# SudhirNikam/cobrix

Measured on AMD Instinct MI355X. Metric: decoded input GB/s + records/s, fixed-len COMP-3 mix, 1-8 MI355X; % HBM peak, higher is better.
Workload: dtype u8; 1 GPU; SYN200: fixed-length 200-byte EBCDIC records, numeric mix (COMP, COMP-3, zoned DISPLAY overpunch, IBM COMP-2, cp037 X(18)) -- BASELINE config C2; records_per_gpu=50000000, input_bytes_per_gpu=10000000000, job_input_bytes=10000000000, output_columns=28, parallelism=dp1, string_layout=Arrow string views (16 B views + long payloads, one pass), occurs_layout=Arrow lists (present elements only), inputs_resident_in_hbm=True

## Files before the change

### cobrix_amd/csrc/cbx_capi.hip

```cpp
#include <hip/hip_runtime.h>

#include <algorithm>
#include <cstdio>
#include <cstring>
#include <functional>
#include <string>
#include <vector>

#include "cbx_kernels.hip"
#include "cbx_select.h"
#include "cbx_text.h"
#include "cbx_hier.h"
#include "cbx_walk.h"
#include "cbx_chain.h"
#include "cbx_filter.h"

using namespace cbx;

static thread_local std::string g_err;

static int fail(int code, const std::string& msg) {
    g_err = msg;
    return code;
}
// ... 58 lines not shown
    std::vector<int32_t> seq_field, seq_slot;
    std::vector<int64_t> seq_tile_cap;
    std::vector<SeqCall> h_seqcall;
    std::vector<int64_t> h_seq_scratch;
    SeqCall* d_seqcall = nullptr;
    uint32_t* d_str_tot = nullptr;  int64_t str_tot_cap = 0;
    int64_t* d_str_excl = nullptr;  int64_t str_excl_cap = 0;
    int64_t* d_block_sums = nullptr; int64_t block_sums_cap = 0;
    uint32_t* d_local = nullptr;    int64_t local_cap = 0;
    uint8_t* d_scratch = nullptr;   int64_t scratch_cap = 0;
    uint64_t* d_stamps = nullptr;
    int64_t jit_min = 262144;
    bool jit_tried[4 * kPre + 5] = {};
    hipFunction_t jit_fn[4 * kPre + 5] = {};
    bool jit_coop[4 * kPre + 5] = {};
    int rec_extent = 0;
    std::string jit_error;
    int last_kind = 0;
    int32_t* d_status = nullptr;
    int num_cus = 256;
    bool walk = false;
    int32_t walk_root = 0, walk_var = 0, walk_n_handlers = 0, walk_depth = 1, walk_max_rec = 0;
    cbx_walk_node* d_wnodes = nullptr;
    std::vector<cbx_walk_node> h_wnodes;
    std::vector<cbx_walk_array> h_warr;
    bool walk_jit_tried = false;
    hipFunction_t walk_jit_fn = nullptr;
    bool chain_jit_tried = false;
    hipFunction_t chain_jit_fn[5] = {};
    bool last_chain_jit = false;
// ... 480 lines not shown
                       (const int64_t*)P->d_block_sums, P->d_str_excl);
    HIP_CHECK(hipGetLastError());
    return CBX_OK;
}

struct CallShape {
    const uint8_t* data; int64_t data_len; const int64_t* rec_off; const int32_t* rec_len;
    int64_t n_rec; int32_t stride; int32_t start_off; int64_t first_record_id;
    const int64_t* rec_id = nullptr;
    const int32_t* rec_seg = nullptr;
    int32_t file_id = -1;
};

static int jit_pro(const cbx_plan* P) { return (P->opts.has_segments ? 1 : 0) | (P->harrays.empty() ? 0 : 2); }

static int launch(cbx_plan* P, const CallShape& c, const cbx_column* columns, int mode, hipStream_t st) {
    const int64_t n_tiles = (c.n_rec + kWave - 1) / kWave;
    KernelArgs a{};
    uintptr_t addr = (uintptr_t)c.data;
    a.base_shift = (int64_t)(addr & 15);
    a.data = (const uint8_t*)(addr & ~(uintptr_t)15);
    a.data_len = c.data_len + a.base_shift;
    a.rec_off = c.rec_off;
    a.rec_len = c.rec_len;
    a.n_rec = c.n_rec;
    a.n_tiles = n_tiles;
    a.pitch = n_tiles * kWave;
    a.stride = c.stride;
    a.start_off = c.start_off;
    a.first_record_id = c.first_record_id;
// ... 201 lines not shown
    hipFunction_t jfn = span_fn;
    int jk = -1;
    if (!span && mode == 0 && P->jit_min >= 0 && c.n_rec >= P->jit_min) {
        const int k = contig ? contig_kp(sdw) : 0;
        if (!P->jit_tried[k]) {
            P->jit_tried[k] = true;
            size_t elems = S.sops.size();
            for (const NumOp& o : S.nops) elems += o.run > 1 ? o.run : 1;
            if (elems > (size_t)kJitMaxOps || S.win.size() > (size_t)kJitMaxWindows)
                P->jit_error = "layout has " + std::to_string(elems) + " elements in " + std::to_string(S.win.size()) +
                               " windows, above the specialised-kernel limits (" + std::to_string(kJitMaxOps) + ", " +
                               std::to_string(kJitMaxWindows) + ")";
            else {
                CoopSplit cs;
                P->jit_coop[k] = jit_coop_of(contig, span, jit_pro(P), str_layout_of(P), S.win, S.nops, S.batches, S.sops, false, &cs);
                P->jit_fn[k] = jit_get(jit_source(contig, k, jit_pro(P), str_layout_of(P), S.win, S.nops, S.batches, S.sops, false), &P->jit_error);
            }
        }
        jfn = P->jit_fn[k];
        jk = k;
    }
    P->last_kind = jfn ? 1 : 0;
    const bool coop = jfn && jk >= 0 && P->jit_coop[jk];
    const size_t lds = coop ? kLutLds + (size_t)a.lds_rows + (size_t)kWavesPerBlock * (a.lds_wave - a.lds_rows) : lds_own;
    if (lds > 160 * 1024) return fail(CBX_E_UNSUPPORTED, "record window does not fit in LDS");
    int blocks_per_cu = (int)std::max<size_t>(1, std::min<size_t>(16, (160 * 1024) / lds));
    int occ = 0;
    const hipError_t oe = jfn ? hipModuleOccupancyMaxActiveBlocksPerMultiprocessor(&occ, jfn, kWave * kWavesPerBlock, lds)
                              : hipOccupancyMaxActiveBlocksPerMultiprocessor(&occ, decode_kernel, kWave * kWavesPerBlock, lds);
    if (oe == hipSuccess && occ > 0) blocks_per_cu = std::min(blocks_per_cu, occ);
    if (!coop && contig && S.sops.size() >= S.nops.size() && S.sops.size() > 0) blocks_per_cu = std::min(blocks_per_cu, 4);
    if (const char* e = getenv("CBX_MAX_BLOCKS_PER_CU")) blocks_per_cu = std::max(1, std::min(blocks_per_cu, atoi(e)));
    const bool piped = P->pipe_peer && mode == 0 && P->packed && P->n_seq > 0;
    if (piped && P->pipe_decode_bpc > 0) blocks_per_cu = std::min(blocks_per_cu, P->pipe_decode_bpc);
    const int64_t blocks_needed = coop ? n_tiles : (n_tiles + kWavesPerBlock - 1) / kWavesPerBlock;
    const int64_t grid = std::min<int64_t>(blocks_needed, (int64_t)P->num_cus * blocks_per_cu);
    const bool prof = P->profiling && mode == 0;
    cbx_plan::CallEvents ce{{nullptr, nullptr, nullptr}};
    if (piped && P->pipe_peer->pipe_done) HIP_CHECK(hipStreamWaitEvent(st, P->pipe_peer->pipe_done, 0));
    if (prof) {
        for (auto& e : ce.e) if (!(e = take_event(P))) return fail(CBX_E_HIP, "hipEventCreate failed");
        HIP_CHECK(hipEventRecord(ce.e[0], st));
    }
    hipFunction_t cfn = nullptr;
    int ck = 0;
    if (mode == 0 && P->packed && P->n_seq > 0 && (contig || span) && P->jit_min >= 0 && c.n_rec >= P->jit_min) {
        const int kp = contig ? contig_kp(sdw) : span_kp;
        const int k = (contig ? 2 : 3) * (kPre + 1) + kp;
        if (!P->jit_tried[k]) {
            P->jit_tried[k] = true;
            std::string err;
            CoopSplit cs;
            P->jit_coop[k] = jit_coop_of(true, span, jit_pro(P), 2, S.win, S.nops, S.batches, S.sops, true, &cs);
            P->jit_fn[k] = jit_get(jit_source(true, kp, jit_pro(P), 2, S.win, S.nops, S.batches, S.sops, span, true),
                                   &err, "cbx_jit_count");
        }
        cfn = P->jit_fn[k];
        ck = k;
    }
    if (mode == 0 && P->packed && P->n_seq > 0 && !cfn && !contig) {
        const int kind = P->last_kind;
        if ((r = launch(P, c, columns, 1, st))) return r;
        P->last_kind = kind;
        if (piped) HIP_CHECK(hipEventRecord(P->pipe_done, st));
    } else if (mode == 0 && P->packed && P->n_seq > 0) {
        KernelArgs ac = a;
        ac.mode = 1;
        size_t clds = lds_own;
        const bool ccoop = cfn && P->jit_coop[ck];
        if (cfn) {
            ac.lds_wave = (a.lds_rows + a.lds_counts + 16 + 15) & ~15;
            clds = 1024 + kLutLds + (ccoop ? (size_t)a.lds_rows + (size_t)kWavesPerBlock * (ac.lds_wave - a.lds_rows)
                                           : (size_t)kWavesPerBlock * ac.lds_wave);
// ... 1868 lines not shown
```

### cobrix_amd/csrc/cbx_decode.h

```cpp
#pragma once
#ifndef __HIPCC_RTC__
#include <hip/hip_runtime.h>
#include <stdint.h>
#endif

#include "cobrix_hip.h"

#define CBX_HD __host__ __device__ __forceinline__
#define CBX_HD_NOINLINE __host__ __device__ __attribute__((noinline))

namespace cbx {

struct U128 {
    uint64_t lo, hi;
};

CBX_HD U128 u128(uint64_t lo, uint64_t hi = 0) { return U128{lo, hi}; }

CBX_HD uint64_t mulhi64(uint64_t a, uint64_t b) {
#if defined(__HIP_DEVICE_COMPILE__)
    return __umul64hi(a, b);
#else
    return (uint64_t)(((unsigned __int128)a * b) >> 64);
#endif
// ... 971 lines not shown
    }
}

constexpr int kStrFastBytes = 32;

CBX_HD void img_bytes32(const uint8_t* img, uint32_t addr, int size, uint32_t w[8]) {
    const uint32_t* p = (const uint32_t*)(img + (addr & ~3u));
    const uint32_t sh = addr & 3u;
    uint32_t r[9];
#pragma unroll
    for (int k = 0; k < 9; k++) r[k] = 4 * k < size + 3 ? p[k] : 0u;
#pragma unroll
    for (int k = 0; k < 8; k++) w[k] = align_bytes(r[k + 1], r[k], sh);
}

CBX_HD uint32_t ctz32(uint32_t x) { return (uint32_t)__builtin_ctz(x); }
CBX_HD uint32_t clz32(uint32_t x) { return (uint32_t)__builtin_clz(x); }
CBX_HD uint32_t popc32(uint32_t x) { return (uint32_t)__builtin_popcount(x); }
CBX_HD uint32_t bits_below(int k) { return k >= 32 ? 0xFFFFFFFFu : ((1u << k) - 1u); }

template <typename LutFn>
CBX_HD void lut_entries32(const uint32_t w[8], int size, LutFn lut, uint32_t ev[kStrFastBytes]) {
#pragma unroll
    for (int j = 0; j < kStrFastBytes; j++) ev[j] = j < size ? lut((w[j >> 2] >> (8 * (j & 3))) & 0xFFu) : 0u;
}

CBX_HD StrSpan string_span32e(int trim, const uint32_t ev[kStrFastBytes], int n, int size) {
    uint32_t keep = 0, m2 = 0, m3 = 0;
#pragma unroll
    for (int j = 0; j < kStrFastBytes; j++) {
// ... 61 lines not shown
```

### cobrix_amd/csrc/cbx_device.h

```cpp
#pragma once
#ifndef __HIPCC_RTC__
#include <hip/hip_runtime.h>
#endif

#include "cbx_internal.h"

#ifndef CBX_DIAG
#define CBX_DIAG 0
#endif

namespace cbx {

__device__ __forceinline__ uint32_t wave_excl_scan32(uint32_t x, int lane, uint32_t& total) {
    uint32_t v = x;
    v += (uint32_t)__builtin_amdgcn_update_dpp(0, (int)v, 0x111, 0xF, 0xF, true);
    v += (uint32_t)__builtin_amdgcn_update_dpp(0, (int)v, 0x112, 0xF, 0xF, true);
    v += (uint32_t)__builtin_amdgcn_update_dpp(0, (int)v, 0x114, 0xF, 0xF, true);
    v += (uint32_t)__builtin_amdgcn_update_dpp(0, (int)v, 0x118, 0xF, 0xF, true);
    const uint32_t r0 = (uint32_t)__builtin_amdgcn_readlane((int)v, 15);
    const uint32_t r1 = (uint32_t)__builtin_amdgcn_readlane((int)v, 31);
    const uint32_t r2 = (uint32_t)__builtin_amdgcn_readlane((int)v, 47);
    const uint32_t r3 = (uint32_t)__builtin_amdgcn_readlane((int)v, 63);
    const int row = lane >> 4;
    v += (row >= 1 ? r0 : 0u) + (row >= 2 ? r1 : 0u) + (row >= 3 ? r2 : 0u);
    total = r0 + r1 + r2 + r3;
    return v - x;
// ... 120 lines not shown
    int avail;
    int seg;
};

template <typename OP>
__device__ __forceinline__ bool odo_present(const CBX_CONST OP* opp, int n_odo, const int32_t* s_cnt, int lane) {
    bool el = true;
    for (int j = 0; j < n_odo; j++) el &= opp->odo_idx[j] < s_cnt[opp->odo_arr[j] * kWave + lane];
    return el;
}

__device__ __forceinline__ uint32_t str_lut(int kind, const uint32_t* s_lut, uint32_t b) {
    return kind == CBX_K_STRING_ASCII ? ascii_lut(b) : s_lut[b];
}

__device__ __forceinline__ StrSpan sop_span(const KernelArgs& a, const StrOp& op, const CBX_CONST StrOp* opp,
                                            const TileCtx& t, const int32_t* s_cnt, int lane, const uint8_t* src,
                                            uint32_t rec_addr, const uint32_t* s_lut, bool& ok, bool fast,
                                            uint32_t ev[kStrFastBytes]) {
    bool el = t.active && (op.segment < 0 || op.segment == t.seg);
    if (op.n_odo) el &= odo_present(opp, op.n_odo, s_cnt, lane);
    const int o = a.start_off + op.eo;
    ok = el && o <= t.avail;
    const int n = ok ? (op.size < t.avail - o ? op.size : t.avail - o) : 0;
    auto lutf = [&](uint32_t b) { return str_lut(op.kind, s_lut, b); };
    if (fast) {
        uint32_t w[8];
        img_bytes32(src, rec_addr + (ok ? (uint32_t)op.eo : 0u), op.size, w);
        lut_entries32(w, op.size, lutf, ev);
        return string_span32e(op.trim, ev, n, op.size);
    }
    StrSpan sp{0, 0, 0};
    if (ok) sp = string_span(op.kind, op.trim, src + rec_addr + (uint32_t)op.eo, n, lutf);
    return sp;
}

__device__ __forceinline__ bool sop_fast(const StrOp& op, bool global) {
    return !global && op.size <= kStrFastBytes && (op.kind == CBX_K_STRING || op.kind == CBX_K_STRING_ASCII);
}

template <int W>
__device__ __forceinline__ void store_w(void* values, int64_t tile, int lane, const Val& x, int out_type) {
    const int w = W ? W : (out_type == CBX_O_I32 || out_type == CBX_O_F32 ? 4 : out_type == CBX_O_DEC128 ? 16 : 8);
// ... 177 lines not shown
                    if (kWide) q0[u] = img_le64_ending(src, end - 8);
                }
            }
#pragma unroll
            for (int u = 0; u < kRunU; u++)
                if (r0 + u < run) run_elem<V, W, kOdo>(a, op, a.nops + i, c, r0 + u, t, ok[u], q1[u], q0[u], s_cnt, lane);
        }
    }
}

template <int V, int W, bool kOdo, int N, typename Sink>
__device__ __forceinline__ void num_group(const KernelArgs& a, const NumOp (&op)[N], int i0, const TileCtx& t,
                                          const uint8_t* src, uint32_t rec_addr, const int32_t* s_cnt, int lane, Sink& sk) {
    constexpr bool kWide = V == V_BCD16 || V == V_ZONED16;
    constexpr bool kRead = V != V_GENERIC;
    const int lim = t.active ? t.avail - a.start_off : -1;
    bool ok[N];
    uint64_t r1[N], r0[N];
#pragma unroll
    for (int u = 0; u < N; u++) {
        ok[u] = op[u].eo + op[u].size <= lim;
        r1[u] = r0[u] = 0;
        if (kRead) {
            const uint32_t end = rec_addr + (ok[u] ? (uint32_t)op[u].eo : 0u) + op[u].size;
            r1[u] = img_le64_ending(src, end);
            if (kWide) r0[u] = img_le64_ending(src, end - 8);
        }
    }
#pragma unroll
    for (int u = 0; u < N; u++) num_one<V, W, kOdo, false>(a, op[u], i0 + u, t, ok[u], r1[u], r0[u], s_cnt, lane, sk);
}

__device__ __forceinline__ uint32_t view_buf(int64_t tile, const StrCall& c) {
// ... 225 lines not shown
        const uint32_t so = __builtin_amdgcn_udot4(lb & 0x02020202u, 0x20100804u, 0u, false);
        nb[g] = __builtin_amdgcn_udot4(lb & 0x03030303u, 0x01010101u, 0u, false);
        wide |= g == 0 ? so >> 3 : so << (4 * g - 3);
        sel[g] = group2_sel(so);
    }
    const int len = (e - b) + (int)popc32(wide & bits_below(e) & ~bits_below(b));
    group2_place(smax, u01, u23, nb, sel, b, len, slot, q, zero_tail);
    return len;
}


__device__ __forceinline__ int str_lane_compose(int kind, int trim, int width, int smax, int eo, int n, bool ok,
                                                const uint8_t* src, uint32_t rec_addr, const uint32_t* s_lut,
                                                uint8_t* s_str, int lane, u32x4 (&q)[kStrNC], bool zero_tail) {
    uint32_t w[8], ev[kStrFastBytes];
    img_bytes32(src, rec_addr + (ok ? (uint32_t)eo : 0u), smax, w);
    const uint32_t lut_a = 0;
    (void)s_lut;
#ifndef CBX_STR_NO_SDWA
    if (kind == CBX_K_STRING) {
#pragma unroll
        for (int j = 0; j < kStrFastBytes; j++)
            ev[j] = j < smax ? lds_ld<uint32_t>(lut_a + ((CBX_DIAG & 32) ? diag_bank(byte_x4(w[j >> 2], j & 3)) : byte_x4(w[j >> 2], j & 3))) : 0u;
    } else {
        lut_entries32(w, smax, [&](uint32_t b) { return ascii_lut(b); }, ev);
    }
#else
    lut_entries32(w, smax, [&](uint32_t b) { return str_lut(kind, s_lut, b); }, ev);
#endif
    uint32_t tr = 0;
#pragma unroll
// ... 58 lines not shown
        }
    }
}

__device__ __forceinline__ u32x4 str_short_view(int len, const u32x4 (&q)[kStrNC]) {
    return u32x4{(uint32_t)len, len > 0 ? q[0].x : 0u, len > 4 ? q[0].y : 0u, len > 8 ? q[0].z : 0u};
}

template <typename Sink>
__device__ __forceinline__ void str_view_fast(const KernelArgs& a, const StrOp& op, const CBX_CONST StrOp* opp, int i,
                                              const StrCall& c, const TileCtx& t, const int32_t* s_cnt,
                                              const uint8_t* src, uint32_t rec_addr, const uint32_t* s_lut,
                                              uint8_t* s_str, int lane, Sink& sk) {
    bool el = t.active && (op.segment < 0 || op.segment == t.seg);
    if (op.n_odo) el &= odo_present(opp, op.n_odo, s_cnt, lane);
    const int o = a.start_off + op.eo;
    const bool ok = el && o <= t.avail;
    const int n = ok ? (op.size < t.avail - o ? op.size : t.avail - o) : 0;
    u32x4 q[kStrNC];
    const int len = str_lane_compose(op.kind, op.trim, op.pad, op.size, op.eo, n, ok, src, rec_addr, s_lut, s_str, lane, q);
    sk.svalid(c, i, t.tile, __ballot(ok));
    const bool lng = len > 12;
    uint32_t tot;
    const uint32_t ex = wave_excl_scan32(lng ? (uint32_t)(len + 3) & ~3u : 0u, lane, tot);
    u32x4 v;
    if (!lng) {
        v = str_short_view(len, q);
    } else {
        str_store_long(gp(c.scratch + t.tile * c.tile_cap + ex), len, op.size * op.pad, q);
        v = u32x4{(uint32_t)len, q[0].x, view_buf(t.tile, c), view_pos(t.tile, c, ex)};
    }
    st_out(gp((u32x4*)c.views) + t.tile * kWave + lane, v);
}

template <typename Sink>
__device__ __forceinline__ void str_view_pair(const KernelArgs& a, const StrOp& A, int ia, const StrCall& ca,
                                              const StrOp& B, int ib, const StrCall& cb, const TileCtx& t,
                                              const uint8_t* src, uint32_t rec_addr, const uint32_t* s_lut,
                                              uint8_t* s_str, int lane, Sink& sk) {
    const bool sa = t.seg == A.segment;
    const int eo = sa ? A.eo : B.eo, size = sa ? A.size : B.size;
    const int smax = A.size > B.size ? A.size : B.size;
    const int o = a.start_off + eo;
    const bool ok = t.active && (sa || t.seg == B.segment) && o <= t.avail;
    const int n = ok ? (size < t.avail - o ? size : t.avail - o) : 0;
    u32x4 q[kStrNC];
    const int len = str_lane_compose(A.kind, A.trim, A.pad, smax, eo, n, ok, src, rec_addr, s_lut, s_str, lane, q);
    sk.svalid(ca, ia, t.tile, __ballot(ok && sa));
    sk.svalid(cb, ib, t.tile, __ballot(ok && !sa));
    const bool lng = len > 12;
    uint32_t tot;
    const uint32_t r4 = lng ? (uint32_t)(len + 3) & ~3u : 0u;
    const uint32_t exb = wave_excl_scan32(sa ? r4 : r4 << 16, lane, tot);
    const uint32_t ex = sa ? exb & 0xFFFFu : exb >> 16;
    u32x4 v;
    if (!lng) {
        v = str_short_view(len, q);
    } else {
// ... 62 lines not shown
    case 3: __builtin_amdgcn_s_waitcnt(0x0F73); break;
    case 4: __builtin_amdgcn_s_waitcnt(0x0F74); break;
    case 5: __builtin_amdgcn_s_waitcnt(0x0F75); break;
    case 6: __builtin_amdgcn_s_waitcnt(0x0F76); break;
    default: __builtin_amdgcn_s_waitcnt(0x0F77); break;
    }
    asm volatile("" ::: "memory");
}


__device__ __forceinline__ int utf8_compose(const KernelArgs& a, const StrOp& op, const CBX_CONST StrOp* opp, const TileCtx& t,
                                            const int32_t* s_cnt, const uint8_t* src, uint32_t rec_addr,
                                            const uint32_t* s_lut, uint8_t* s_str, int lane, bool& ok, u32x4 (&q)[kStrNC]) {
    bool el = t.active && (op.segment < 0 || op.segment == t.seg);
    if (op.n_odo) el &= odo_present(opp, op.n_odo, s_cnt, lane);
    const int o = a.start_off + op.eo;
    ok = el && o <= t.avail;
    const int n = ok ? (op.size < t.avail - o ? op.size : t.avail - o) : 0;
    const int len = str_lane_compose(op.kind, op.trim, op.pad, op.size, op.eo, n, ok, src, rec_addr, s_lut, s_str, lane, q, false);
    return ok ? len : 0;
}

__device__ __forceinline__ int64_t utf8_tile_base(const StrCall& c, const TileCtx& t) {
    const CBX_CONST int64_t* x = (const CBX_CONST int64_t*)c.excl;
    return x[t.tile] - x[0];
}

__device__ __forceinline__ CBX_GLOBAL uint8_t* utf8_offsets(const KernelArgs& a, const StrCall& c, const TileCtx& t, int64_t base,
                                                            uint32_t ex, int len, uint32_t tot, int lane) {
    CBX_GLOBAL int32_t* offs = gp((int32_t*)c.local);
    st_out(offs + t.tile * kWave + lane, (int32_t)(base + ex));
// ... 99 lines not shown
        const uint32_t td = sd[k1];
        CBX_GLOBAL uint8_t* tp = A + 4 * k1;
        if (tb >= 2) st_pay((CBX_GLOBAL uint16_t*)(tp), (uint16_t)td);
        if (tb & 1) tp[tb & 2] = (uint8_t)(td >> (8 * (tb & 2)));
    }
}

struct G2 {
    uint32_t u01[kStrNG], u23[kStrNG], nb[kStrNG];
    uint2 sel[kStrNG];
    int b, e, len;
};

__device__ __forceinline__ void g2_prep(int trim, int smax, int eo, int n, bool ok, const uint8_t* src, uint32_t rec_addr, G2& g) {
    uint32_t w[8], ev[kStrFastBytes];
    img_bytes32(src, rec_addr + (ok ? (uint32_t)eo : 0u), smax, w);
#pragma unroll
    for (int j = 0; j < kStrFastBytes; j++)
        ev[j] = j < smax ? lds_ld<uint32_t>(byte_x4(w[j >> 2], j & 3)) : 0u;
    uint32_t tr = 0;
#pragma unroll
    for (int j = 0; j < kStrFastBytes; j++)
        if (j < smax) tr = __builtin_amdgcn_alignbit(tr, ev[j], 31);
    const uint32_t keep = ~(__builtin_bitreverse32(tr) >> (32 - smax)) & bits_below(n);
    int b = 0, e = n;
    if (trim == CBX_TRIM_LEFT || trim == CBX_TRIM_BOTH) b = keep ? (int)ctz32(keep) : n;
    if (trim == CBX_TRIM_RIGHT || trim == CBX_TRIM_BOTH) e = keep ? 32 - (int)clz32(keep) : b;
    uint32_t wide = 0;
#pragma unroll
    for (int q = 0; q < kStrNG; q++) {
        if (4 * q >= smax) break;
// ... 65 lines not shown
    __builtin_amdgcn_s_waitcnt(0xC07F);
    const uint32_t q_lo = ph ? 1u : 0u, q_hi = end >> 4;
    for (uint32_t q = q_lo + (uint32_t)lane; q < q_hi; q += kWave)
        st_pay((CBX_GLOBAL u32x4*)(A + 16u * q), lds_ld<u32x4>(sb + 16u * q));
    const uint32_t he = end < 16u ? end : 16u;
    if (ph && (uint32_t)lane >= ph && (uint32_t)lane < he) A[lane] = lds_ld<uint8_t>(sb + (uint32_t)lane);
    const uint32_t t0 = 16u * q_hi;
    if (t0 >= 16u * q_lo && t0 + (uint32_t)lane < end && (t0 > 0 || !ph)) A[t0 + lane] = lds_ld<uint8_t>(sb + t0 + (uint32_t)lane);
}

__device__ __forceinline__ void str_utf8_fast2(const KernelArgs& a, const StrOp& op, const CBX_CONST StrOp* opp,
                                               const StrCall& c, const TileCtx& t, const int32_t* s_cnt,
                                               const uint8_t* src, uint32_t rec_addr, uint8_t* s_str, int lane) {
    bool el = t.active && (op.segment < 0 || op.segment == t.seg);
    if (op.n_odo) el &= odo_present(opp, op.n_odo, s_cnt, lane);
    const int o = a.start_off + op.eo;
    const bool ok = el && o <= t.avail;
    const int n = ok ? (op.size < t.avail - o ? op.size : t.avail - o) : 0;
    G2 g;
    g2_prep(op.trim, op.size, op.eo, n, ok, src, rec_addr, g);
    gp(c.validity)[t.tile] = __ballot(ok);
    uint32_t tot;
    const uint32_t ex = wave_excl_scan32((uint32_t)g.len, lane, tot);
    CBX_GLOBAL uint8_t* dst = utf8_offsets(a, c, t, utf8_tile_base(c, t), ex, g.len, tot, lane);
    if (!dst || (CBX_DIAG & 16)) return;
#ifndef CBX_U8_DIRECT
    g2_stage_store(dst, ex, tot, op.size, g, true, s_str, lane);
#else
    g2_store(dst + ex, op.size, g, s_str, lane);
#endif
}
// ... 44 lines not shown

__device__ __forceinline__ void str_utf8_two(const KernelArgs& a, const StrOp& A, const CBX_CONST StrOp* oppA, const StrCall& ca,
                                             const StrOp& B, const CBX_CONST StrOp* oppB, const StrCall& cb,
                                             const TileCtx& t, const int32_t* s_cnt, const uint8_t* src, uint32_t rec_addr,
                                             const uint32_t* s_lut, uint8_t* s_str, int lane) {
    str_utf8_two(a, A, oppA, ca, B, oppB, cb, t, s_cnt, src, rec_addr, s_lut, s_str, lane, utf8_tile_base(ca, t),
                 utf8_tile_base(cb, t));
}

__device__ __forceinline__ void str_utf8_pair(const KernelArgs& a, const StrOp& A, const StrCall& ca, const StrOp& B,
                                              const StrCall& cb, const TileCtx& t, const uint8_t* src, uint32_t rec_addr,
                                              const uint32_t* s_lut, uint8_t* s_str, int lane) {
    const bool sa = t.seg == A.segment;
    const int eo = sa ? A.eo : B.eo, size = sa ? A.size : B.size;
    const int smax = A.size > B.size ? A.size : B.size;
    const int o = a.start_off + eo;
    const bool ok = t.active && (sa || t.seg == B.segment) && o <= t.avail;
    const int n = ok ? (size < t.avail - o ? size : t.avail - o) : 0;
    const bool g2 = A.kind == CBX_K_STRING && A.pad == 2;
    G2 g;
    u32x4 q[kStrNC];
    int len;
    if (g2) {
        g2_prep(A.trim, smax, eo, n, ok, src, rec_addr, g);
        len = g.len;
    } else {
        const int l0 = str_lane_compose(A.kind, A.trim, A.pad, smax, eo, n, ok, src, rec_addr, s_lut, s_str, lane, q, false);
        len = ok ? l0 : 0;
    }
    gp(ca.validity)[t.tile] = __ballot(ok && sa);
    gp(cb.validity)[t.tile] = __ballot(ok && !sa);
// ... 12 lines not shown
        return;
    }
#endif
    if (!d) return;
    if (g2) g2_store(d, smax, g, s_str, lane);
    else utf8_store_direct(d, len, smax * A.pad, q);
}

__device__ __forceinline__ uint8_t count_lut_byte(uint32_t e) {
    return (uint8_t)(((e >> 31) << 7) | ((e >> 24) & 3u));
}

__device__ __forceinline__ int str_count_lane(int trim, int smax, int size, int eo, const uint8_t* src, uint32_t rec_addr, bool ok,
                                              const uint32_t* s_lut) {
    uint32_t w[8];
    img_bytes32(src, rec_addr + (ok ? (uint32_t)eo : 0u), smax, w);
    uint32_t acc = 0, tm = 0;
    const uint32_t lut8 = lds_addr(s_lut);
#pragma unroll
    for (int j = 0; j < kStrFastBytes; j++) {
        if (j < smax) {
            const uint32_t idx = (w[j >> 2] >> (8 * (j & 3))) & 0xFFu;
            const uint32_t e = (uint32_t)(int32_t)lds_ld<int8_t>(lut8 + idx);
            tm = __builtin_amdgcn_alignbit(tm, e, 31);
            acc += j < size ? (e & 0xFFu) : 0u;
        }
    }
    const uint32_t keep = ~__builtin_bitreverse32(tm << (32 - smax)) & bits_below(size);
    const int total = (int)(acc & 127u);
    const bool tl = trim == CBX_TRIM_LEFT || trim == CBX_TRIM_BOTH;
    const bool tr = trim == CBX_TRIM_RIGHT || trim == CBX_TRIM_BOTH;
    if (!ok) return 0;
    if (!keep) return (tl || tr) ? 0 : total;
    const int lead = (int)ctz32(keep), trail = size - (32 - (int)clz32(keep));
    return total - (tl ? lead : 0) - (tr ? trail : 0);
}

__device__ __forceinline__ int str_count_fast(const StrOp& op, const uint8_t* src, uint32_t rec_addr, bool ok,
                                              const uint32_t* s_lut) {
    uint32_t w[8];
    img_bytes32(src, rec_addr + (ok ? (uint32_t)op.eo : 0u), op.size, w);
    uint32_t acc = 0;
    const uint32_t lut8 = lds_addr(s_lut);
    const int size = op.size;
#ifndef CBX_COUNT_B64
    uint32_t tm = 0;
#pragma unroll
    for (int j = 0; j < kStrFastBytes; j++) {
        if (j < size) {
            const uint32_t idx = (w[j >> 2] >> (8 * (j & 3))) & 0xFFu;
            const uint32_t e = (uint32_t)(int32_t)lds_ld<int8_t>(lut8 + ((CBX_DIAG & 32) ? diag_bank(idx) : idx));
            tm = __builtin_amdgcn_alignbit(tm, e, 31);
            acc += e & 0xFFu;
        }
    }
    const uint32_t keep = ~__builtin_bitreverse32(tm << (32 - size)) & bits_below(size);
// ... 22 lines not shown
#endif
    const int total = (int)(acc & 127u);
    const bool tl = op.trim == CBX_TRIM_LEFT || op.trim == CBX_TRIM_BOTH;
    const bool tr = op.trim == CBX_TRIM_RIGHT || op.trim == CBX_TRIM_BOTH;
    if (!ok) return 0;
    if (!keep) return (tl || tr) ? 0 : total;
    const int lead = (int)ctz32(keep), trail = size - (32 - (int)clz32(keep));
    return total - (tl ? lead : 0) - (tr ? trail : 0);
}

__device__ __forceinline__ bool str_count_pair(const KernelArgs& a, const StrOp& A, const StrOp& B, const TileCtx& t,
                                               const uint8_t* src, uint32_t rec_addr, const uint32_t* s_lut, int lane) {
    const bool sa = t.seg == A.segment;
    const int eo = sa ? A.eo : B.eo, size = sa ? A.size : B.size;
    const int smax = A.size > B.size ? A.size : B.size;
    const int o = a.start_off + eo;
    const bool el = t.active && (sa || t.seg == B.segment);
    const bool ok = el && o + size <= t.avail;
    const bool part = el && o <= t.avail && !ok;
    if (A.kind != CBX_K_STRING || __ballot(part)) return false;
    const int len = str_count_lane(A.trim, smax, size, eo, src, rec_addr, ok, s_lut + 256);
    const uint32_t la = sa ? (uint32_t)len : 0u, lb = sa ? 0u : (uint32_t)len;
    uint32_t tot2;
    wave_excl_scan32(la | (lb << 16), lane, tot2);
    if (lane == 0) {
        gp(a.str_tot)[(int64_t)A.seq * a.n_tiles + t.tile] = tot2 & 0xFFFFu;
        gp(a.str_tot)[(int64_t)B.seq * a.n_tiles + t.tile] = tot2 >> 16;
    }
    return true;
}

// ... 6 lines not shown
    const bool fast = sop_fast(op, global);
    if (kView && fast) {
        DirectSink ds;
        if (sk) str_view_fast(a, op, opp, i, c, t, s_cnt, src, rec_addr, s_lut, s_str, lane, *sk);
        else str_view_fast(a, op, opp, i, c, t, s_cnt, src, rec_addr, s_lut, s_str, lane, ds);
        return;
    }
    if (!kView && fast && str_layout(a) == 2 && kmode(a) == 0) {
        str_utf8_fast(a, op, opp, c, t, s_cnt, src, rec_addr, s_lut, s_str, lane);
        return;
    }
#ifdef CBX_COUNT_LUT
    if (!kView && fast && op.kind == CBX_K_STRING) {
        bool el = t.active && (op.segment < 0 || op.segment == t.seg);
        if (op.n_odo) el &= odo_present(opp, op.n_odo, s_cnt, lane);
        const int o = a.start_off + op.eo;
        const bool ok = el && o + op.size <= t.avail;
        const bool part = el && o <= t.avail && !ok;
        if (!__ballot(part)) {
            uint32_t tot;
            wave_excl_scan32((uint32_t)str_count_fast(op, src, rec_addr, ok, s_lut + 256), lane, tot);
            if (lane == 0) gp(a.str_tot)[(int64_t)op.seq * a.n_tiles + t.tile] = tot;
            return;
        }
    }
#endif
    bool ok;
    uint32_t ev[kStrFastBytes];
    const StrSpan sp = sop_span(a, op, opp, t, s_cnt, lane, src, rec_addr, s_lut, ok, fast, ev);
    if (kView) {
        DirectSink ds;
// ... 258 lines not shown
}

template <bool kFramed = true>
__device__ __forceinline__ TileCtx tile_ctx(const KernelArgs& a, int64_t tile, int lane) {
    TileCtx t;
    t.tile = tile;
    t.rec = tile * kWave + lane;
    t.active = t.rec < a.n_rec;
    t.base = a.base_shift;
    t.avail = 0;
    t.seg = -1;
    if (kFramed && a.rec_off) {
        if (t.active) { t.base += a.rec_off[t.rec]; t.avail = a.rec_len[t.rec]; }
    } else if (t.active) {
        t.base += t.rec * (int64_t)a.stride;
        t.avail = a.stride;
    }
    return t;
}

template <bool kSel = true, bool kSeg = true, bool kArr = true>
__device__ __forceinline__ void tile_prologue(const KernelArgs& a, TileCtx& t, const uint8_t* rp, int lane,
                                              const uint32_t* s_lut, int32_t* s_cnt) {
    if (kSel && a.rec_seg) t.seg = t.active ? a.rec_seg[t.rec] : -1;
    else if (kSeg && a.segmap && t.active) t.seg = segment_of(a, s_lut, rp, t.avail);
    if (kSeg && kmode(a) == 0 && a.seg_col >= 0) {
        const DevColumn c = ldc(a.cols + a.seg_col);
        if (t.active) gp((int32_t*)c.values)[t.rec] = t.seg;
        const uint64_t m = __ballot(t.active);
        if (lane == 0) gp(c.validity)[t.tile] = m;
    }
// ... 123 lines not shown
    uint4 buf[KP];
    tile = first_tile<Body>(tile);
    if (tile < a.n_tiles) contig_issue<KP>(a, contig_span(a, tile), lane, buf);
    Stamps st;
    st.init();
    while (tile < a.n_tiles) {
        const ContigSpan sp = contig_span(a, tile);
        contig_store<KP>(a, sp, lane, buf, l.img);
        wave_sync_lds();
        st.mark(0);
        const int64_t next = next_tile<Body>(tile, tstep);
        body.begin(tile);
        if (!kLate) contig_issue<KP>(a, contig_span(a, next), lane, buf);
        st.mark(1);
        TileCtx t = tile_ctx<false>(a, tile, lane);
        const uint32_t rec0 = (uint32_t)(lane * a.cpitch + 4 * sp.mis_dw);
        tile_prologue<false, (kPro & 1) != 0, (kPro & 2) != 0>(a, t, l.img + rec0, lane, l.lut, l.cnt);
        st.mark(2);
        body.pre(a, t, (const uint8_t*)l.img, rec0 + (uint32_t)a.start_off, l, lane, st);
        if (kLate) contig_issue<KP>(a, contig_span(a, next), lane, buf);
        body.post(a, t, (const uint8_t*)l.img, rec0 + (uint32_t)a.start_off, l, lane, st);
        run_end(a, body, tile, lane);
        wave_sync_lds();
        st.mark(5);
        tile = next;
    }
    st.flush(a, lane);
}

template <int KP>
__device__ __forceinline__ void coop_issue(const KernelArgs& a, const ContigSpan& sp, int wid, int lane,
                                           uint4 (&buf)[(KP + kWavesPerBlock - 1) / kWavesPerBlock]) {
    constexpr int KH = (KP + kWavesPerBlock - 1) / kWavesPerBlock;
    int64_t left = a.data_len - sp.a0;
    left = left < 0 ? 0 : (left > (1 << 20) ? (1 << 20) : left);
    const uint64_t base = (uint64_t)(a.data + sp.a0);
// ... 38 lines not shown
    tile = first_tile<Body>(tile);
    if (tile >= a.n_tiles) return;
    coop_issue<KP>(a, contig_span(a, tile), wid, lane, buf);
    coop_put<KP>(a, contig_span(a, tile), wid, lane, buf, l.img);
    Stamps st;
    st.init();
    while (true) {
        __syncthreads();
        st.mark(0);
        const ContigSpan sp = contig_span(a, tile);
        const int64_t next = next_tile<Body>(tile, tstep);
        body.begin(tile);
        coop_issue<KP>(a, contig_span(a, next), wid, lane, buf);
        st.mark(1);
        TileCtx t = tile_ctx<false>(a, tile, lane);
        const uint32_t rec0 = (uint32_t)(lane * a.cpitch + 4 * sp.mis_dw);
        st.mark(2);
        body.template part<kW>(a, t, (const uint8_t*)l.img, rec0 + (uint32_t)a.start_off, l, lane, st);
        run_end(a, body, tile, lane);
        __syncthreads();
        st.mark(5);
        tile = next;
        if (tile >= a.n_tiles) break;
        coop_put<KP>(a, contig_span(a, tile), wid, lane, buf, l.img);
    }
    st.flush(a, lane);
}

__device__ __forceinline__ void span_recs(const KernelArgs& a, int64_t tile, int lane, int64_t& off, int32_t& len) {
    const int64_t r = tile * kWave + lane;
    const int64_t rc = r < a.n_rec ? r : a.n_rec - 1;
    const int64_t o = a.rec_off[rc];
    const int32_t l = a.rec_len[rc];
// ... 105 lines not shown
```

### cobrix_amd/csrc/cbx_internal.h

```cpp
#pragma once
#ifndef __HIPCC_RTC__
#include <hip/hip_runtime.h>
#include <stdint.h>
#endif

#include "cbx_decode.h"
#include "cobrix_hip.h"

#define CBX_CONST __attribute__((address_space(4)))

namespace cbx {

constexpr int kWave = 64;
constexpr int kWavesPerBlock = 2;
constexpr int kGuard = 16;
constexpr int kLutLds = 1024 + 128;
constexpr int kMaxWindowBytes = 1024;
constexpr int kStrStageBytes = 4096;
constexpr int kMaxStrItems = 256;

struct StrOp {
    int32_t eo;
    int32_t size;
    uint8_t kind, trim, n_odo, pad;
// ... 105 lines not shown
    const CBX_CONST DevColumn* cols;
    int32_t n_seq;
    uint32_t* str_tot;
    int32_t* status;
    int32_t* list_len;
    int32_t* list_flag;
    uint64_t* defer_bits;
    int32_t lds_rows;
    int32_t lds_counts;
    int32_t str_stage;
    int32_t lds_wave;
    int32_t dump_stride;
    uint64_t* stamps;
};

}
```

### cobrix_amd/csrc/cbx_jit.h

```cpp
#pragma once
#include <hip/hiprtc.h>

#include <algorithm>
#include <cstdlib>
#include <map>
#include <mutex>
#include <sstream>
#include <string>
#include <utility>
#include <vector>

#include "cbx_jit_src.inc"

namespace cbx {

constexpr int kJitMaxStrUnroll = 16;

static std::string jit_u64(uint64_t v) {
    std::ostringstream o;
    o << "0x" << std::hex << v << "ull";
    return o.str();
}

static void jit_numop(std::ostringstream& o, const NumOp& n) {
// ... 197 lines not shown
    bool runs = false;
    for (const NumOp& op : nops) n_defer = std::max(n_defer, op.defer + 1);
    for (const Batch& b : batches) runs |= b.runs != 0;
    *n_str_words = layout == 1 && getenv("CBX_STR_VWORDS") ? (int)sops.size() : 0;
    return (count || runs || span || getenv("CBX_NO_VWORDS")) ? 0 : (int)nops.size() + n_defer + *n_str_words;
}

static bool jit_coop_of(bool contig, bool span, int pro, int layout, const std::vector<Window>& win, const std::vector<NumOp>& nops,
                        const std::vector<Batch>& batches, const std::vector<StrOp>& sops, bool count, CoopSplit* out) {
    int nsw = 0;
    const int nw = contig ? jit_words(layout, nops, batches, sops, span, count, &nsw) : 0;
    return jit_coop(contig, span, pro, win, nops, batches, sops, count, nw, nsw, out);
}

static std::string jit_source(bool contig, int kp, int pro, int layout, const std::vector<Window>& win, const std::vector<NumOp>& nops,
                              const std::vector<Batch>& batches, const std::vector<StrOp>& sops, bool span, bool count = false) {
    std::ostringstream o;
    const bool view = layout == 1;
    if (const char* d = getenv("CBX_JIT_DEFINES")) {
        std::string s(d);
        for (size_t b = 0; b < s.size();) {
            size_t e = s.find(',', b);
            if (e == std::string::npos) e = s.size();
            std::string m = s.substr(b, e - b);
            const size_t q = m.find('=');
            if (!m.empty()) o << "#define " << (q == std::string::npos ? m : m.substr(0, q) + " " + m.substr(q + 1)) << "\n";
            b = e + 1;
        }
    }
    if (getenv("CBX_STR_NO_SHIFT")) o << "#define CBX_STR_NO_SHIFT 1\n";
    o << "#define CBX_STR_LAYOUT " << layout << "\n";
    o << "#define CBX_MODE " << (count ? 1 : 0) << "\n";
// ... 273 lines not shown
```

Before: 2719 GB/s.

## Specialise JIT decode and count kernels on static record geometry

Adds a small per-plan cache of JIT kernels compiled with record stride, LDS pitch and start offset baked in as compile-time constants. String byte gathers can then use constant-offset loads, and the address arithmetic folds away. The decode kernel is specialised only for string-only layouts, while the count kernel is specialised whenever the batch is contiguous. The cost is extra runtime compilations, up to four per kernel kind, when geometry varies.

```diff
diff --git a/cobrix_amd/csrc/cbx_capi.hip b/cobrix_amd/csrc/cbx_capi.hip
--- a/cobrix_amd/csrc/cbx_capi.hip
+++ b/cobrix_amd/csrc/cbx_capi.hip
@@ -96,6 +96,10 @@
     bool jit_tried[4 * kPre + 5] = {};
     hipFunction_t jit_fn[4 * kPre + 5] = {};
     bool jit_coop[4 * kPre + 5] = {};
+    struct JitStatic { JitGeo geo; hipFunction_t fn = nullptr; };
+    std::vector<JitStatic> jit_geo[4 * kPre + 5];
+    bool jit_spec[4 * kPre + 5] = {};
+    bool jit_gen_tried[4 * kPre + 5] = {};
     int rec_extent = 0;
     std::string jit_error;
     int last_kind = 0;
@@ -606,6 +610,18 @@
 
 static int jit_pro(const cbx_plan* P) { return (P->opts.has_segments ? 1 : 0) | (P->harrays.empty() ? 0 : 2); }
 
+template <typename Src>
+static hipFunction_t jit_static(cbx_plan* P, int k, const JitGeo& geo, const char* name, std::string* err, Src src) {
+    for (const cbx_plan::JitStatic& e : P->jit_geo[k])
+        if (e.geo == geo) return e.fn;
+    if ((int)P->jit_geo[k].size() >= kJitMaxGeo) return nullptr;
+    cbx_plan::JitStatic e;
+    e.geo = geo;
+    e.fn = jit_get(src(&e.geo), err, name);
+    P->jit_geo[k].push_back(e);
+    return e.fn;
+}
+
 static int launch(cbx_plan* P, const CallShape& c, const cbx_column* columns, int mode, hipStream_t st) {
     const int64_t n_tiles = (c.n_rec + kWave - 1) / kWave;
     KernelArgs a{};
@@ -837,11 +853,21 @@
             else {
                 CoopSplit cs;
                 P->jit_coop[k] = jit_coop_of(contig, span, jit_pro(P), str_layout_of(P), S.win, S.nops, S.batches, S.sops, false, &cs);
+                P->jit_spec[k] = true;
+            }
+        }
+        jk = k;
+        if (P->jit_spec[k] && contig && S.nops.empty())
+            jfn = jit_static(P, k, JitGeo{a.stride, a.cpitch, a.start_off}, "cbx_jit_decode", &P->jit_error, [&](const JitGeo* g) {
+                return jit_source(true, k, jit_pro(P), str_layout_of(P), S.win, S.nops, S.batches, S.sops, false, false, g);
+            });
+        if (P->jit_spec[k] && !jfn) {
+            if (!P->jit_gen_tried[k]) {
+                P->jit_gen_tried[k] = true;
                 P->jit_fn[k] = jit_get(jit_source(contig, k, jit_pro(P), str_layout_of(P), S.win, S.nops, S.batches, S.sops, false), &P->jit_error);
             }
-        }
-        jfn = P->jit_fn[k];
-        jk = k;
+            jfn = P->jit_fn[k];
+        }
     }
     P->last_kind = jfn ? 1 : 0;
     const bool coop = jfn && jk >= 0 && P->jit_coop[jk];
@@ -872,14 +898,24 @@
         const int k = (contig ? 2 : 3) * (kPre + 1) + kp;
         if (!P->jit_tried[k]) {
             P->jit_tried[k] = true;
-            std::string err;
             CoopSplit cs;
             P->jit_coop[k] = jit_coop_of(true, span, jit_pro(P), 2, S.win, S.nops, S.batches, S.sops, true, &cs);
-            P->jit_fn[k] = jit_get(jit_source(true, kp, jit_pro(P), 2, S.win, S.nops, S.batches, S.sops, span, true),
-                                   &err, "cbx_jit_count");
-        }
-        cfn = P->jit_fn[k];
+        }
         ck = k;
+        std::string cerr;
+        if (contig)
+            cfn = jit_static(P, k, JitGeo{a.stride, a.cpitch, a.start_off}, "cbx_jit_count", &cerr, [&](const JitGeo* g) {
+                return jit_source(true, kp, jit_pro(P), 2, S.win, S.nops, S.batches, S.sops, false, true, g);
+            });
+        if (!cfn) {
+            if (!P->jit_gen_tried[k]) {
+                P->jit_gen_tried[k] = true;
+                std::string err;
+                P->jit_fn[k] = jit_get(jit_source(true, kp, jit_pro(P), 2, S.win, S.nops, S.batches, S.sops, span, true),
+                                       &err, "cbx_jit_count");
+            }
+            cfn = P->jit_fn[k];
+        }
     }
     if (mode == 0 && P->packed && P->n_seq > 0 && !cfn && !contig) {
         const int kind = P->last_kind;
diff --git a/cobrix_amd/csrc/cbx_decode.h b/cobrix_amd/csrc/cbx_decode.h
--- a/cobrix_amd/csrc/cbx_decode.h
+++ b/cobrix_amd/csrc/cbx_decode.h
@@ -1009,6 +1009,21 @@
     for (int k = 0; k < 8; k++) w[k] = align_bytes(r[k + 1], r[k], sh);
 }
 
+CBX_HD void img_bytes32_at(const uint8_t* rec, int off, int size, uint32_t w[8]) {
+    const uint32_t* p = (const uint32_t*)rec + (off >> 2);
+    const uint32_t sh = (uint32_t)off & 3u;
+    uint32_t r[9];
+#pragma unroll
+    for (int k = 0; k < 9; k++) r[k] = 4 * k < size + 3 ? p[k] : 0u;
+#pragma unroll
+    for (int k = 0; k < 8; k++) w[k] = sh == 0 ? r[k] : align_bytes(r[k + 1], r[k], sh);
+}
+template <int OFF, int SIZE>
+CBX_HD void img_bytes32_c(const uint8_t* rec, uint32_t w[8]) {
+    static_assert(OFF >= 0 && SIZE >= 0 && SIZE <= kStrFastBytes, "a register-path string element");
+    img_bytes32_at(rec, OFF, SIZE, w);
+}
+
 CBX_HD uint32_t ctz32(uint32_t x) { return (uint32_t)__builtin_ctz(x); }
 CBX_HD uint32_t clz32(uint32_t x) { return (uint32_t)__builtin_clz(x); }
 CBX_HD uint32_t popc32(uint32_t x) { return (uint32_t)__builtin_popcount(x); }
diff --git a/cobrix_amd/csrc/cbx_device.h b/cobrix_amd/csrc/cbx_device.h
--- a/cobrix_amd/csrc/cbx_device.h
+++ b/cobrix_amd/csrc/cbx_device.h
@@ -10,6 +10,21 @@
 #endif
 
 namespace cbx {
+
+#if defined(CBX_GEO_STRIDE)
+constexpr bool kGeoStatic = true;
+constexpr int kGeoStride = CBX_GEO_STRIDE, kGeoCpitch = CBX_GEO_CPITCH, kGeoStart = CBX_GEO_START, kGeoLim = CBX_GEO_LIM;
+static_assert(kGeoStride > 0 && kGeoStride % 4 == 0 && kGeoCpitch % 4 == 0 && kGeoCpitch >= kGeoStride &&
+              kGeoLim == kGeoStride - kGeoStart, "static geometry of a contiguous fixed-length batch");
+#else
+constexpr bool kGeoStatic = false;
+constexpr int kGeoStride = 0, kGeoCpitch = 0, kGeoStart = 0, kGeoLim = 0;
+#endif
+__device__ __forceinline__ int geo_stride(const KernelArgs& a) { return kGeoStatic ? kGeoStride : a.stride; }
+__device__ __forceinline__ int geo_cpitch(const KernelArgs& a) { return kGeoStatic ? kGeoCpitch : a.cpitch; }
+__device__ __forceinline__ int geo_start(const KernelArgs& a) { return kGeoStatic ? kGeoStart : a.start_off; }
+__device__ __forceinline__ constexpr bool geo_fits(int eo, int size) { return kGeoStatic && eo >= 0 && eo + size <= kGeoLim; }
+__device__ __forceinline__ const uint8_t* geo_rec(const uint8_t* src, uint32_t rec_addr) { return src + (rec_addr - (uint32_t)kGeoStart); }
 
 __device__ __forceinline__ uint32_t wave_excl_scan32(uint32_t x, int lane, uint32_t& total) {
     uint32_t v = x;
@@ -160,19 +175,24 @@
     return kind == CBX_K_STRING_ASCII ? ascii_lut(b) : s_lut[b];
 }
 
+__device__ __forceinline__ void str_bytes32(const uint8_t* src, uint32_t rec_addr, bool ok, int eo, int size, uint32_t w[8]) {
+    if (geo_fits(eo, size)) img_bytes32_at(geo_rec(src, rec_addr), kGeoStart + eo, size, w);
+    else img_bytes32(src, rec_addr + (ok ? (uint32_t)eo : 0u), size, w);
+}
+
 __device__ __forceinline__ StrSpan sop_span(const KernelArgs& a, const StrOp& op, const CBX_CONST StrOp* opp,
                                             const TileCtx& t, const int32_t* s_cnt, int lane, const uint8_t* src,
                                             uint32_t rec_addr, const uint32_t* s_lut, bool& ok, bool fast,
                                             uint32_t ev[kStrFastBytes]) {
     bool el = t.active && (op.segment < 0 || op.segment == t.seg);
     if (op.n_odo) el &= odo_present(opp, op.n_odo, s_cnt, lane);
-    const int o = a.start_off + op.eo;
+    const int o = geo_start(a) + op.eo;
     ok = el && o <= t.avail;
     const int n = ok ? (op.size < t.avail - o ? op.size : t.avail - o) : 0;
     auto lutf = [&](uint32_t b) { return str_lut(op.kind, s_lut, b); };
     if (fast) {
         uint32_t w[8];
-        img_bytes32(src, rec_addr + (ok ? (uint32_t)op.eo : 0u), op.size, w);
+        str_bytes32(src, rec_addr, ok, op.eo, op.size, w);
         lut_entries32(w, op.size, lutf, ev);
         return string_span32e(op.trim, ev, n, op.size);
     }
@@ -380,9 +400,9 @@
                                           const uint8_t* src, uint32_t rec_addr, const int32_t* s_cnt, int lane, Sink& sk) {
     constexpr bool kWide = V == V_BCD16 || V == V_ZONED16;
     constexpr bool kRead = V != V_GENERIC;
-    const int lim = t.active ? t.avail - a.start_off : -1;
     bool ok[N];
     uint64_t r1[N], r0[N];
+    const int lim = t.active ? t.avail - a.start_off : -1;
 #pragma unroll
     for (int u = 0; u < N; u++) {
         ok[u] = op[u].eo + op[u].size <= lim;
@@ -638,7 +658,7 @@
                                                 const uint8_t* src, uint32_t rec_addr, const uint32_t* s_lut,
                                                 uint8_t* s_str, int lane, u32x4 (&q)[kStrNC], bool zero_tail) {
     uint32_t w[8], ev[kStrFastBytes];
-    img_bytes32(src, rec_addr + (ok ? (uint32_t)eo : 0u), smax, w);
+    str_bytes32(src, rec_addr, ok, eo, smax, w);
     const uint32_t lut_a = 0;
     (void)s_lut;
 #ifndef CBX_STR_NO_SDWA
@@ -727,7 +747,7 @@
                                               uint8_t* s_str, int lane, Sink& sk) {
     bool el = t.active && (op.segment < 0 || op.segment == t.seg);
     if (op.n_odo) el &= odo_present(opp, op.n_odo, s_cnt, lane);
-    const int o = a.start_off + op.eo;
+    const int o = geo_start(a) + op.eo;
     const bool ok = el && o <= t.avail;
     const int n = ok ? (op.size < t.avail - o ? op.size : t.avail - o) : 0;
     u32x4 q[kStrNC];
@@ -754,7 +774,7 @@
     const bool sa = t.seg == A.segment;
     const int eo = sa ? A.eo : B.eo, size = sa ? A.size : B.size;
     const int smax = A.size > B.size ? A.size : B.size;
-    const int o = a.start_off + eo;
+    const int o = geo_start(a) + eo;
     const bool ok = t.active && (sa || t.seg == B.segment) && o <= t.avail;
     const int n = ok ? (size < t.avail - o ? size : t.avail - o) : 0;
     u32x4 q[kStrNC];
@@ -847,7 +867,7 @@
                                             const uint32_t* s_lut, uint8_t* s_str, int lane, bool& ok, u32x4 (&q)[kStrNC]) {
     bool el = t.active && (op.segment < 0 || op.segment == t.seg);
     if (op.n_odo) el &= odo_present(opp, op.n_odo, s_cnt, lane);
-    const int o = a.start_off + op.eo;
+    const int o = geo_start(a) + op.eo;
     ok = el && o <= t.avail;
     const int n = ok ? (op.size < t.avail - o ? op.size : t.avail - o) : 0;
     const int len = str_lane_compose(op.kind, op.trim, op.pad, op.size, op.eo, n, ok, src, rec_addr, s_lut, s_str, lane, q, false);
@@ -977,7 +997,7 @@
 
 __device__ __forceinline__ void g2_prep(int trim, int smax, int eo, int n, bool ok, const uint8_t* src, uint32_t rec_addr, G2& g) {
     uint32_t w[8], ev[kStrFastBytes];
-    img_bytes32(src, rec_addr + (ok ? (uint32_t)eo : 0u), smax, w);
+    str_bytes32(src, rec_addr, ok, eo, smax, w);
 #pragma unroll
     for (int j = 0; j < kStrFastBytes; j++)
         ev[j] = j < smax ? lds_ld<uint32_t>(byte_x4(w[j >> 2], j & 3)) : 0u;
@@ -1073,7 +1093,7 @@
                                                const uint8_t* src, uint32_t rec_addr, uint8_t* s_str, int lane) {
     bool el = t.active && (op.segment < 0 || op.segment == t.seg);
     if (op.n_odo) el &= odo_present(opp, op.n_odo, s_cnt, lane);
-    const int o = a.start_off + op.eo;
+    const int o = geo_start(a) + op.eo;
     const bool ok = el && o <= t.avail;
     const int n = ok ? (op.size < t.avail - o ? op.size : t.avail - o) : 0;
     G2 g;
@@ -1148,7 +1168,7 @@
     const bool sa = t.seg == A.segment;
     const int eo = sa ? A.eo : B.eo, size = sa ? A.size : B.size;
     const int smax = A.size > B.size ? A.size : B.size;
-    const int o = a.start_off + eo;
+    const int o = geo_start(a) + eo;
     const bool ok = t.active && (sa || t.seg == B.segment) && o <= t.avail;
     const int n = ok ? (size < t.avail - o ? size : t.avail - o) : 0;
     const bool g2 = A.kind == CBX_K_STRING && A.pad == 2;
@@ -1191,7 +1211,7 @@
 __device__ __forceinline__ int str_count_lane(int trim, int smax, int size, int eo, const uint8_t* src, uint32_t rec_addr, bool ok,
                                               const uint32_t* s_lut) {
     uint32_t w[8];
-    img_bytes32(src, rec_addr + (ok ? (uint32_t)eo : 0u), smax, w);
+    str_bytes32(src, rec_addr, ok, eo, smax, w);
     uint32_t acc = 0, tm = 0;
     const uint32_t lut8 = lds_addr(s_lut);
 #pragma unroll
@@ -1216,7 +1236,7 @@
 __device__ __forceinline__ int str_count_fast(const StrOp& op, const uint8_t* src, uint32_t rec_addr, bool ok,
                                               const uint32_t* s_lut) {
     uint32_t w[8];
-    img_bytes32(src, rec_addr + (ok ? (uint32_t)op.eo : 0u), op.size, w);
+    str_bytes32(src, rec_addr, ok, op.eo, op.size, w);
     uint32_t acc = 0;
     const uint32_t lut8 = lds_addr(s_lut);
     const int size = op.size;
@@ -1269,7 +1289,7 @@
     const bool sa = t.seg == A.segment;
     const int eo = sa ? A.eo : B.eo, size = sa ? A.size : B.size;
     const int smax = A.size > B.size ? A.size : B.size;
-    const int o = a.start_off + eo;
+    const int o = geo_start(a) + eo;
     const bool el = t.active && (sa || t.seg == B.segment);
     const bool ok = el && o + size <= t.avail;
     const bool part = el && o <= t.avail && !ok;
@@ -1306,7 +1326,7 @@
     if (!kView && fast && op.kind == CBX_K_STRING) {
         bool el = t.active && (op.segment < 0 || op.segment == t.seg);
         if (op.n_odo) el &= odo_present(opp, op.n_odo, s_cnt, lane);
-        const int o = a.start_off + op.eo;
+        const int o = geo_start(a) + op.eo;
         const bool ok = el && o + op.size <= t.avail;
         const bool part = el && o <= t.avail && !ok;
         if (!__ballot(part)) {
@@ -1595,7 +1615,7 @@
         if (t.active) { t.base += a.rec_off[t.rec]; t.avail = a.rec_len[t.rec]; }
     } else if (t.active) {
         t.base += t.rec * (int64_t)a.stride;
-        t.avail = a.stride;
+        t.avail = geo_stride(a);
     }
     return t;
 }
@@ -1749,12 +1769,12 @@
         if (!kLate) contig_issue<KP>(a, contig_span(a, next), lane, buf);
         st.mark(1);
         TileCtx t = tile_ctx<false>(a, tile, lane);
-        const uint32_t rec0 = (uint32_t)(lane * a.cpitch + 4 * sp.mis_dw);
+        const uint32_t rec0 = (uint32_t)(lane * geo_cpitch(a) + 4 * sp.mis_dw);
         tile_prologue<false, (kPro & 1) != 0, (kPro & 2) != 0>(a, t, l.img + rec0, lane, l.lut, l.cnt);
         st.mark(2);
-        body.pre(a, t, (const uint8_t*)l.img, rec0 + (uint32_t)a.start_off, l, lane, st);
+        body.pre(a, t, (const uint8_t*)l.img, rec0 + (uint32_t)geo_start(a), l, lane, st);
         if (kLate) contig_issue<KP>(a, contig_span(a, next), lane, buf);
-        body.post(a, t, (const uint8_t*)l.img, rec0 + (uint32_t)a.start_off, l, lane, st);
+        body.post(a, t, (const uint8_t*)l.img, rec0 + (uint32_t)geo_start(a), l, lane, st);
         run_end(a, body, tile, lane);
         wave_sync_lds();
         st.mark(5);
@@ -1823,9 +1843,9 @@
         coop_issue<KP>(a, contig_span(a, next), wid, lane, buf);
         st.mark(1);
         TileCtx t = tile_ctx<false>(a, tile, lane);
-        const uint32_t rec0 = (uint32_t)(lane * a.cpitch + 4 * sp.mis_dw);
+        const uint32_t rec0 = (uint32_t)(lane * geo_cpitch(a) + 4 * sp.mis_dw);
         st.mark(2);
-        body.template part<kW>(a, t, (const uint8_t*)l.img, rec0 + (uint32_t)a.start_off, l, lane, st);
+        body.template part<kW>(a, t, (const uint8_t*)l.img, rec0 + (uint32_t)geo_start(a), l, lane, st);
         run_end(a, body, tile, lane);
         __syncthreads();
         st.mark(5);
diff --git a/cobrix_amd/csrc/cbx_internal.h b/cobrix_amd/csrc/cbx_internal.h
--- a/cobrix_amd/csrc/cbx_internal.h
+++ b/cobrix_amd/csrc/cbx_internal.h
@@ -143,4 +143,10 @@
     uint64_t* stamps;
 };
 
+struct JitGeo {
+    int stride = 0, cpitch = 0, start_off = 0;
+    bool operator==(const JitGeo& g) const { return stride == g.stride && cpitch == g.cpitch && start_off == g.start_off; }
+};
+constexpr int kJitMaxGeo = 4;
+
 }
diff --git a/cobrix_amd/csrc/cbx_jit.h b/cobrix_amd/csrc/cbx_jit.h
--- a/cobrix_amd/csrc/cbx_jit.h
+++ b/cobrix_amd/csrc/cbx_jit.h
@@ -235,8 +235,12 @@
 }
 
 static std::string jit_source(bool contig, int kp, int pro, int layout, const std::vector<Window>& win, const std::vector<NumOp>& nops,
-                              const std::vector<Batch>& batches, const std::vector<StrOp>& sops, bool span, bool count = false) {
+                              const std::vector<Batch>& batches, const std::vector<StrOp>& sops, bool span, bool count = false,
+                              const JitGeo* geo = nullptr) {
     std::ostringstream o;
+    if (geo && contig && !span)
+        o << "#define CBX_GEO_STRIDE " << geo->stride << "\n#define CBX_GEO_CPITCH " << geo->cpitch << "\n#define CBX_GEO_START "
+          << geo->start_off << "\n#define CBX_GEO_LIM " << geo->stride - geo->start_off << "\n";
     const bool view = layout == 1;
     if (const char* d = getenv("CBX_JIT_DEFINES")) {
         std::string s(d);
```

New measurement: 2614 GB/s. -3.9%, worse.
